# iastro-pt/gpyrn

Measured on AMD Instinct MI355X. Metric: ELBO iterations/sec (N=4096, P=3, Q=2), higher is better.
Workload: dtype f64; 1 GPU; BASELINE config 3: N=4096, p=3 outputs, q=2 nodes, QP nodes / SE weights, synthetic RV series (seed 0); latent_gps=8, comm_ranks=1

## Files before the change

gpyrn_amd/csrc/api.hip:

```cpp
#include "api_internal.h"

#include <dlfcn.h>
#include <fcntl.h>
#include <pthread.h>
#include <sched.h>
#include <sys/mman.h>
#include <sys/stat.h>
#include <time.h>
#include <unistd.h>
#include <atomic>
#include <math.h>
#include <rccl/rccl.h>
#include <stdlib.h>
#include <string.h>

#include <algorithm>

static hipEvent_t prof_event(gprn_ctx* c)
{
    if (!c->prof.pool.empty()) {
        hipEvent_t e = c->prof.pool.back();
        c->prof.pool.pop_back();
        return e;
    }
// ... 123 lines not shown
    if (!c || !name) return GPRN_E_ARG;
    int* field = nullptr;
    if (!strcmp(name, "flags")) { factor_use_flags(c); field = &c->use_flags; }
    else if (!strcmp(name, "wait_budget_ms")) field = &c->wait_budget_ms;
    else if (!strcmp(name, "withhold_inner")) field = &c->withhold_inner;
    else if (!strcmp(name, "overlap")) field = &c->overlap_opt;
    else if (!strcmp(name, "small_path")) field = &c->small_opt;
    else if (!strcmp(name, "bulk_pad_kb")) field = &c->pad_kb_opt;
    else if (!strcmp(name, "small_pad_kb")) field = &c->pad_small_kb_opt;
    else if (!strcmp(name, "batch_mem_mb")) field = &c->batch_mem_mb;
    else if (!strcmp(name, "batch_mask")) field = &c->batch_mask;
    else if (!strcmp(name, "order_mask")) field = &c->order_mask;
    else if (!strcmp(name, "grad_exact")) field = &c->grad_exact;
    else if (!strcmp(name, "elbo_form")) field = &c->elbo_form;
    else if (!strcmp(name, "predict_form")) field = &c->predict_form;
    else if (!strcmp(name, "state_ready")) { if (old) *old = c->grad_ready ? 1 : 0; return GPRN_OK; }
    else if (!strcmp(name, "comm_budget_s")) field = &c->comm_budget_s;
    else if (!strcmp(name, "accurate_factor")) field = &c->acc_opt;
    else if (!strcmp(name, "fenced_finalize")) field = &c->fenced_finalize;
    else if (!strcmp(name, "fallbacks")) { if (old) *old = c->fallbacks; return GPRN_OK; }
    else if (!strcmp(name, "batch_chunk")) { if (old) *old = c->last_batch_chunk; return GPRN_OK; }
    else return bad(c, "set_option: unknown option");
    if (old) *old = *field;
    const bool is_pad = field == &c->pad_kb_opt || field == &c->pad_small_kb_opt;
    if ((is_pad || field == &c->acc_opt) && value == -2) { *field = -1; return GPRN_OK; }
    if (field == &c->predict_form && value < -1)
        return bad(c, "set_option: predict_form is GPRN_PREDICT_REFERENCE or GPRN_PREDICT_POSTERIOR");
    if (value >= 0) {
        if (field == &c->use_flags && value) {
            int can = 0;
            if (hipDeviceGetAttribute(&can, hipDeviceAttributeCanUseStreamWaitValue, c->device) != hipSuccess) can = 0;
            if (!can) return bad(c, "set_option: this device has no stream memory operations");
        }
        if (field == &c->wait_budget_ms && value < 1) return bad(c, "set_option: wait_budget_ms >= 1");
        if (field == &c->batch_mem_mb && value < 1) return bad(c, "set_option: batch_mem_mb >= 1");
        if (field == &c->comm_budget_s && value < 1) return bad(c, "set_option: comm_budget_s >= 1");
        if (field == &c->batch_mask && value > 1) return bad(c, "set_option: batch_mask is 0 or 1");
        if (field == &c->order_mask && value > 1) return bad(c, "set_option: order_mask is 0 or 1");
        if (field == &c->order_mask && !value && c->d_mask && c->sweep_order != GPRN_ORDER_REFERENCE) {
            c->err = "set_option: order_mask stays 1 while a data mask (gprn_set_mask) and the sequential sweep order "
                     "(gprn_set_sweep_order) are both in force";
            return GPRN_E_UNSUPPORTED;
        }
        if (field == &c->grad_exact && value > 1) return bad(c, "set_option: grad_exact is 0 or 1");
        if (field == &c->predict_form) {
            if (value != GPRN_PREDICT_REFERENCE && value != GPRN_PREDICT_POSTERIOR)
                return bad(c, "set_option: predict_form is GPRN_PREDICT_REFERENCE or GPRN_PREDICT_POSTERIOR");
            if (value == GPRN_PREDICT_POSTERIOR && (c->comm || c->shm || c->world > 1)) {
                c->err = "set_option: the posterior form of prediction is not supported on a context with a communicator";
                return GPRN_E_UNSUPPORTED;
            }
        }
        if (field == &c->elbo_form) {
            if (value != GPRN_ELBO_REFERENCE && value != GPRN_ELBO_BOUND) return bad(c, "set_option: elbo_form is GPRN_ELBO_REFERENCE or GPRN_ELBO_BOUND");
            if (value == GPRN_ELBO_BOUND && (c->comm || c->shm || c->world > 1)) {
                c->err = "set_option: the bound form of the ELBO is not supported on a context with a communicator";
                return GPRN_E_UNSUPPORTED;
            }
// ... 39 lines not shown
    HIP_TRY(c, hipMemset(c->d_info, 0, 3 * (size_t)nslot * sizeof(int)));
    c->nslot = nslot;
    return GPRN_OK;
}

void free_problem(gprn_ctx* c)
{
    dev_free(c->d_time); dev_free(c->d_yraw); dev_free(c->d_yerr2); dev_free(c->d_yres);
    dev_free(c->d_variance); dev_free(c->d_mu); dev_free(c->d_var);
    dev_free(c->d_mu_save); dev_free(c->d_var_save);
    dev_free(c->d_mu_alt); dev_free(c->d_var_alt);
    dev_free(c->d_mu_old); c->mu_old_cap = 0;
    if (c->d_loop_ctl) { hipFree(c->d_loop_ctl); c->d_loop_ctl = nullptr; }
    small_batch_free(c);
    mid_batch_free(c);
    if (c->grad_scratch) { hipFree(c->grad_scratch); c->grad_scratch = nullptr; c->grad_scratch_bytes = 0; }
    if (c->h_pin_in) { hipHostFree(c->h_pin_in); c->h_pin_in = nullptr; c->pin_in_cap = 0; }
    if (c->h_pin_out) { hipHostFree(c->h_pin_out); c->h_pin_out = nullptr; c->pin_out_cap = 0; }
    dev_free(c->d_loop_hist);
    for (auto& p : c->K) dev_free(p);
    for (auto& p : c->KLinv) dev_free(p);
    for (auto& p : c->Kinv) dev_free(p);
    for (auto& p : c->Sig) dev_free(p);
    for (auto& p : c->wsB) dev_free(p);
    for (auto& p : c->wsX) dev_free(p);
    c->K.clear(); c->KLinv.clear(); c->Kinv.clear(); c->Sig.clear(); c->wsB.clear(); c->wsX.clear();
    dev_free(c->d_logdetK);
    dev_free(c->d_kinv_tab); dev_free(c->d_kinv_out); dev_free(c->d_small_ticket); dev_free(c->d_small_stamps);
    for (auto& p : c->predKs) dev_free(p);
    for (auto& p : c->predWT) dev_free(p);
// ... 59 lines not shown
{
    if (!out) return GPRN_E_ARG;
    *out = nullptr;
    int n = 0;
    if (hipGetDeviceCount(&n) != hipSuccess || n <= 0) return GPRN_E_NODEV;
    if (device_id < 0 || device_id >= n) return GPRN_E_ARG;
    if (hipSetDevice(device_id) != hipSuccess) return GPRN_E_HIP;
    gprn_ctx* c = new gprn_ctx();
    c->device = device_id;
    c->shared = device_streams_acquire(device_id);
    if (!c->shared) { delete c; return GPRN_E_HIP; }
    c->stream = c->shared->s[0];
    c->stream2 = c->shared->s[1];
    c->stream3 = c->shared->s[2];
    c->stream4 = c->shared->s[3];
    if (hipEventCreateWithFlags(&c->ev_diag, hipEventDisableTiming) != hipSuccess ||
        hipEventCreateWithFlags(&c->ev_first, hipEventDisableTiming) != hipSuccess ||
        hipEventCreateWithFlags(&c->ev_minil, hipEventDisableTiming) != hipSuccess ||
        hipEventCreateWithFlags(&c->ev_inner, hipEventDisableTiming) != hipSuccess ||
        hipEventCreateWithFlags(&c->ev_panel, hipEventDisableTiming) != hipSuccess ||
        hipEventCreateWithFlags(&c->ev_rest, hipEventDisableTiming) != hipSuccess ||
        hipEventCreateWithFlags(&c->ev_resta, hipEventDisableTiming) != hipSuccess ||
        hipEventCreateWithFlags(&c->ev_next, hipEventDisableTiming) != hipSuccess ||
        hipEventCreateWithFlags(&c->ev_nodes, hipEventDisableTiming) != hipSuccess ||
        hipEventCreateWithFlags(&c->ev_tail, hipEventDisableTiming) != hipSuccess ||
        hipEventCreateWithFlags(&c->ev_q1, hipEventDisableTiming) != hipSuccess) {
        device_streams_release(c->shared);
        delete c;
        return GPRN_E_HIP;
    }
// ... 648 lines not shown
```

gpyrn_amd/csrc/api_sweep.hip:

```cpp
#include "api_internal.h"

static int factor_priors_impl(gprn_ctx* c);

extern "C" int gprn_factor_priors(gprn_ctx* c)
{
    DeviceLock lock_(c);
    WatchScope watch_(c, "gprn_factor_priors");
    if (!c || !c->N) return bad(c, "factor_priors: call set_data first");
    HIP_TRY(c, hipSetDevice(c->device));
    if (c->owner.empty()) return bad(c, "factor_priors: call set_owners first");
    c->grad_ready = false;
    int pre = GPRN_OK;
    for (int g = 0; g < c->G && !pre; ++g)
        if (!c->kspec[g].set) pre = bad(c, "factor_priors: a latent GP has no kernel");
    if ((pre = agree_to_start(c, pre, "factor_priors"))) return pre;
    return with_event_fallback(c, "factor_priors", [&](bool) { return factor_priors_impl(c); }, true);
}

static int ensure_small_sweep_tabs(gprn_ctx* c)
{
    if (c->small_sweep_ready) return GPRN_OK;
    std::vector<double*> ktab(c->q, nullptr);
    for (int j = 1; j < c->q && c->elbo_form == GPRN_ELBO_REFERENCE; ++j) {
        if (!c->Kinv[j]) return bad(c, "small path: K_j^-1 of a node is missing (no set-up yet?)");
// ... 200 lines not shown
static int small_sweep(gprn_ctx* c, const double* mu_in, const double* var_in, double* mu_out, double* var_out,
                       double* out4, double* scal, const SmallLoop* loop)
{
    c->d_scal = scal;
    const int* done = loop ? loop->ctl : nullptr;
    TRY(ensure_small_sweep_tabs(c));
    TRY(small_phase(c, sweep_phase(c, false), false, scal, mu_in, var_in, mu_out, var_out, done));
    TRY(order_small(c, sweep_phase(c, false), false, mu_in, var_in, mu_out, var_out, done));
    TRY(mask_rows(c, sweep_phase(c, false), false, mu_out, var_out, done));
    TRY(small_phase(c, sweep_phase(c, true), true, scal, mu_in, var_in, mu_out, var_out, done));
    TRY(order_small(c, sweep_phase(c, true), true, mu_in, var_in, mu_out, var_out, done));
    TRY(mask_rows(c, sweep_phase(c, true), true, mu_out, var_out, done));
    return small_tail(c, out4, scal, mu_out, var_out, loop);
}

int phase_core(gprn_ctx* c, const Phase& ph, bool weights, double* scal, std::function<int()>& chain_started)
{
    const size_t o = (size_t)ph.slot0 * ph.ld;
    TRY(order_snapshot(c, ph));
    TRY(vec_prep(c, ph, weights));
    const int overlap = overlap_mask(c);
    FactorHooks h;
    h.build_B = true;
    h.ft_s = (overlap & 1) ? c->d_s + o : nullptr;
    if (overlap & 2) {
        h.rows_final = [c, &ph, o](int r0, int r1, hipStream_t st) -> int {
            TRY(vec_lower_matvec(c, ph, BUF_X, c->d_z + o, ph.ld, 0, c->d_u + o, st, r0 * GPRN_TILE, (r1 - r0) * GPRN_TILE));
            return vec_colops_partial(c, ph, st, r0, r1 - r0);
        };
    }
    h.chain_started.swap(chain_started);
    const int rc_f = factor_invert(c, ph, false, &h);
    chain_started.swap(h.chain_started);
    TRY(rc_f);
    TRY(vec_lower_matvec(c, ph, BUF_X, c->d_z + o, ph.ld, 0, c->d_u + o, nullptr, h.rows_done * GPRN_TILE, -1));
    TRY(vec_colops_partial(c, ph, nullptr, h.rows_done, -1));
    if (overlap & 8) TRY(vec_reduce_finalize(c, ph, scal, true));
    else {
        TRY(vec_colops_reduce(c, ph));
        TRY(vec_logdet(c, ph, BUF_B, scal));
        TRY(vec_finalize(c, ph, scal, false));
    }
    TRY(order_refresh(c, ph, weights));
    return mask_rows(c, ph, weights, c->d_mu, c->d_var, nullptr);
}

static int mu_k_mu(gprn_ctx* c, bool weights, double* out, hipStream_t stream = nullptr)
{
    const Phase ph = sweep_phase(c, weights);
    if (!ph.nslots) return GPRN_OK;
    double* a = c->d_u + (size_t)ph.slot0 * ph.ld;
    TRY(vec_lower_matvec(c, ph, BUF_KLINV, c->d_mu, c->N, c->elbo_form == GPRN_ELBO_BOUND ? 2 : 1, a, stream));
    return vec_dot_self(c, ph, a, out, stream);
}

struct NodeSide {
    std::function<int()> work;
    bool q1 = false;
    bool term_done = false;
};

static int run_phase(gprn_ctx* c, bool weights, double* scal, std::function<int()>& handed, NodeSide* nodes)
{
    const Phase ph = sweep_phase(c, weights);
    const std::vector<int>& gps = weights ? c->loc_weights : c->loc_nodes;
    const int ns = ph.nslots;
    const size_t o = (size_t)ph.slot0 * ph.ld;
    if (ns) {
        TRY(phase_core(c, ph, weights, scal, handed));
        const int overlap = overlap_mask(c);
        if (c->keep_sigma) {
            const size_t nn = (size_t)c->ld * c->ld;
            TRY(lauum_lower(c, ph));
            for (int s = 0; s < ns; ++s) {
                if (!c->Sig[gps[s]]) {
                    TRY(dev_alloc(c, &c->Sig[gps[s]], nn));
                    HIP_TRY(c, hipMemsetAsync(c->Sig[gps[s]], 0, nn * sizeof(double), c->stream));
                }
                TRY(vec_sigma(c, c->wsB[ph.slot0 + s], c->d_s + o + (size_t)s * c->ld, c->Sig[gps[s]]));
            }
        }
        const bool bound = c->elbo_form == GPRN_ELBO_BOUND;
        if (!weights && c->q > 1 && (!bound || ((overlap & 4) && !c->loc_weights.empty()))) {
            Phase inv = ph;
            inv.nslots = (gps.back() == c->q - 1) ? ns - 1 : ns;
            const std::vector<int> node_gps = gps;
            const std::vector<double*> node_B(c->wsB.begin(), c->wsB.begin() + ns);
            HIP_TRY(c, hipEventRecord(c->ev_nodes, c->stream));
            const bool early_term = (overlap & 4) && !c->loc_weights.empty();
            nodes->term_done = early_term;
            nodes->q1 = true;
            nodes->work = [c, scal, early_term, inv, node_gps, node_B, bound]() -> int {
                HIP_TRY(c, hipStreamWaitEvent(c->stream2, c->ev_nodes, 0));
                if (early_term) TRY(mu_k_mu(c, false, scal + 2 * (size_t)c->G, c->stream2));
                if (inv.nslots && !c->keep_sigma && !bound) TRY(lauum_lower(c, inv, c->stream2));
                for (size_t s = 0; s < node_gps.size() && !bound; ++s) {
                    const int k = node_gps[s];
                    for (int j = k + 1; j < c->q; ++j)
                        TRY(vec_q1(c, c->Kinv[j], node_B[s], c->d_s + s * c->ld, c->d_u,
                                   scal + 3 * (size_t)c->G + (size_t)j * c->q + k, c->stream2));
                }
                HIP_TRY(c, hipEventRecord(c->ev_q1, c->stream2));
                return GPRN_OK;
            };
        }
    }
    if (handed) {
        std::function<int()> f;
        f.swap(handed);
        TRY(f());
    }
    return exchange_rows(c, weights);
}

// ... 458 lines not shown
```

gpyrn_amd/csrc/factor.hip:

```cpp
#include "gprn_internal.h"
#include "tile_mma.h"
#include "diag_tile.h"
#include "vecops.h"

#include <math.h>
#include <stdlib.h>

#include <algorithm>
#include <functional>

template <bool ARGS, bool ACC>
__global__ __launch_bounds__(256) __attribute__((amdgpu_waves_per_eu(1, 1)))
void k_diag_block(double* const* __restrict__ ptrs, PtrArgs pa, int ld, int kblk, int* __restrict__ info,
                  unsigned* sig_slot, unsigned sig_value, const unsigned* wait_flag, unsigned wait_value,
                  unsigned* wait_timed_out, int nph)
{
    __shared__ __attribute__((aligned(16))) double lds[ACC ? DIAG_LDS_DOUBLES_ACC : DIAG_LDS_DOUBLES];
    if (pa.stamps && blockIdx.x == 0 && threadIdx.x == 0) pa.stamps[0] = __builtin_amdgcn_s_memrealtime();
    await_flag(wait_flag, wait_value, wait_timed_out);
    if (pa.stamps && blockIdx.x == 0 && threadIdx.x == 0) pa.stamps[1] = __builtin_amdgcn_s_memrealtime();
    const int slot = blockIdx.x;
    const size_t off = ((size_t)kblk * GPRN_TILE) * ld + (size_t)kblk * GPRN_TILE;
    double* const Bm = ARGS ? pa.p[slot][0] : ptrs[(size_t)slot * GPRN_NBUF + BUF_B];
    double* const Xm = ARGS ? pa.p[slot][1] : ptrs[(size_t)slot * GPRN_NBUF + BUF_X];
// ... 154 lines not shown
                auto by_klen = [](const TileTask& a, const TileTask& b) { return a.klen < b.klen; };
                std::stable_sort(v.begin() + begin, v.begin() + begin + na, by_klen);
                std::stable_sort(v.begin() + begin + na, v.end(), by_klen);
                o.rest0 = begin; o.nrest = v.size() - begin; o.nrestA = na;
            }
        }
        outers.push_back(o);
    }
    }
    c->lauum0 = v.size();
    for (int a = T - 1; a >= 0; --a)
        for (int b = 0; b <= a; ++b)
            v.push_back(TileTask{toff(a, b, ld), toff(a, a, ld), toff(a, b, ld), ld - a * GPRN_TILE,
                                 BUF_B, BUF_X, BUF_X, tile_modes(CM_SET, 1, 1)});
    c->nlauum = v.size() - c->lauum0;

    if (v.size() > c->tasks_cap) {
        if (c->d_tasks) hipFree(c->d_tasks);
        c->d_tasks = nullptr;
        HIP_TRY(c, hipMalloc(&c->d_tasks, v.size() * sizeof(TileTask)));
        c->tasks_cap = v.size();
    }
    HIP_TRY(c, hipStreamSynchronize(c->stream2));
    HIP_TRY(c, hipMemcpyAsync(c->d_tasks, v.data(), v.size() * sizeof(TileTask),
                              hipMemcpyHostToDevice, c->stream));
    HIP_TRY(c, hipStreamSynchronize(c->stream));
    c->tasks_T = T;
    return GPRN_OK;
}

// ... 445 lines not shown
        (void)hipStreamSynchronize(c->stream); (void)hipStreamSynchronize(c->stream2);
        (void)hipStreamSynchronize(c->stream3);
        if (c->stream4) (void)hipStreamSynchronize(c->stream4);
        (void)hipMemset(c->d_sig + (size_t)c->sig_T * GPRN_FLAG_KINDS * 2, 0, sizeof(unsigned));
    }
    return rc;
}

int lauum_lower(gprn_ctx* c, const Phase& ph, hipStream_t stream)
{
    int rc = ensure_tasks(c, ph.T);
    if (rc) return rc;
    return launch_tiles(c, c->d_tasks + c->lauum0, c->nlauum, ph.ptrs, ph.nslots, ph.ld,
                        GPRN_T_LAUUM, stream);
}
```

gpyrn_amd/csrc/gemm_tile.hip:

```cpp
#include "gprn_internal.h"

#include <stdlib.h>
#include <string.h>

#include <algorithm>
#include <type_traits>

#include "tile_mma.h"
#include "diag_tile.h"

template <int BM, int BN, int NW, int TRI, int TAG>
__global__ __launch_bounds__(64 * NW, NW == 8 ? 4 : 2)
void k_tile_gemm(const TileTask* __restrict__ tasks, double* const* __restrict__ ptrs, int ld,
                 unsigned* sig_slot, unsigned sig_value, const unsigned* then_wait, unsigned then_value,
                 const unsigned* wait_flag, unsigned wait_value, unsigned* wait_timed_out, int xcd_map,
                 const double* ft_s, int ft_n,
                 unsigned* start_flag, unsigned start_value, int ldc_arg)
{
    if (start_flag && blockIdx.x == 0 && blockIdx.y == 0 && threadIdx.x == 0)
        __hip_atomic_store(start_flag, start_value, __ATOMIC_RELEASE, __HIP_MEMORY_SCOPE_SYSTEM);
    await_flag(wait_flag, wait_value, wait_timed_out);
    constexpr int WM = 2, WN = NW / 2;
    constexpr int SM = GPRN_TILE / BM, SN = GPRN_TILE / BN;
    __shared__ __attribute__((aligned(16))) double lds[2 * 16 * (BM + BN + 32)];
// ... 5 lines not shown
    const unsigned bx = lb % gx, by = lb / gx;
    const TileTask t = tasks[bx / (SM * SN)];
    const int sub = bx % (SM * SN), sr = sub / SN, sc = sub % SN;
    double* const* gp = ptrs + (size_t)by * GPRN_NBUF;
    double* const p0 = gp[0]; double* const p1 = gp[1]; double* const p2 = gp[2]; double* const p3 = gp[3];
    auto pick = [&](int b) { return b == 0 ? p0 : (b == 1 ? p1 : (b == 2 ? p2 : p3)); };
    const int c_mode = t.modes & 3;
    const int a_mode = (t.modes >> 2) & 1;
    const int b_mode = (t.modes >> 3) & 1;
    const double* A = pick(t.a_buf) + t.a_off + (a_mode ? (size_t)sr * BM : (size_t)sr * BM * ld);
    const double* B = pick(t.b_buf) + t.b_off + (b_mode ? (size_t)sc * BN : (size_t)sc * BN * ld);
    const int ldc_own = TAG == TG_COV ? ldc_arg : 0;
    gptr_t C = (gptr_t)(pick(t.c_buf) + t.c_off) + (size_t)sr * BM * (ldc_own ? ldc_own : ld) + sc * BN;

    constexpr bool CAN_LOWER = BM == 64 && BN == 64 && TRI == 0 &&
                               (TAG == TG_INNER || TAG == TG_NEXT || TAG == TG_BULK || TAG == TG_AHEAD || TAG == TG_COV);
    const bool lower = CAN_LOWER && ((t.modes >> 4) & 1);
    constexpr bool CAN_FT = BM == 64 && BN == 64 && TRI == 0 && (TAG == TG_NEXT || TAG == TG_BULK || TAG == TG_AHEAD);
    const double* ft_K = nullptr;
    const double* ft_sv = nullptr;
    int ft_row = 0, ft_col = 0;
    if (CAN_FT && ft_s && ((t.modes >> 5) & 1)) {
        ft_K = pick(BUF_K) + t.c_off + (size_t)sr * BM * ld + sc * BN;
        ft_sv = ft_s + (size_t)by * ld;
        ft_row = (int)(t.c_off / ld) + sr * BM;
        ft_col = (int)(t.c_off % ld) + sc * BN;
    }
    constexpr bool CAN_SYM128 = BM == 128 && BN == 128 && TRI == 0 && (TAG == TG_INNER || TAG == TG_NEXT);
    if (lower && sr < sc) {  }
    else if (CAN_LOWER && lower && sr == sc)
        tile_mma<BM, BN, WM, WN, TRI, CAN_LOWER, true>(lds, A, B, C, ld, a_mode, b_mode, c_mode, t.klen,
                                                       (sr * BM) >> 4, (sc * BN) >> 4, ft_K, ft_sv, ft_row, ft_col, ft_n, ldc_own);
    else if (CAN_SYM128 && ((t.modes >> 4) & 1))
        tile_mma<BM, BN, WM, WN, TRI, false, false, CAN_SYM128>(lds, A, B, C, ld, a_mode, b_mode, c_mode, t.klen,
                                                                (sr * BM) >> 4, (sc * BN) >> 4);
    else
        tile_mma<BM, BN, WM, WN, TRI, false, true>(lds, A, B, C, ld, a_mode, b_mode, c_mode, t.klen,
                                                   (sr * BM) >> 4, (sc * BN) >> 4, ft_K, ft_sv, ft_row, ft_col, ft_n, ldc_own);
    signal_done(sig_slot, sig_value, then_wait, then_value, wait_timed_out);
}

template <bool ACC>
__global__ __launch_bounds__(256, ACC ? 1 : 2)
void k_tile_panel(const TileTask* __restrict__ tasks, int n_l, double* const* __restrict__ ptrs, int ld,
                  unsigned* sig_slot, unsigned sig_value, const unsigned* then_wait, unsigned then_value,
                  unsigned* wait_timed_out, const unsigned* wait_flag, unsigned wait_value,
                  unsigned* start_flag, unsigned start_value, unsigned* start_flag2)
{
    if (blockIdx.x == 0 && blockIdx.y == 0 && threadIdx.x == 0) {
        if (start_flag) __hip_atomic_store(start_flag, start_value, __ATOMIC_RELEASE, __HIP_MEMORY_SCOPE_SYSTEM);
        if (start_flag2) __hip_atomic_store(start_flag2, start_value, __ATOMIC_RELEASE, __HIP_MEMORY_SCOPE_SYSTEM);
    }
// ... 238 lines not shown
    case TS_64x128_BTRI * 8 + TG_PANEL: GO(64, 128, 1, TG_PANEL); break;
    case TS_128x64_ATRI * 8 + TG_PANEL: GO(128, 64, 2, TG_PANEL); break;
    case TS_64x64 * 8 + TG_INNER: GO(64, 64, 0, TG_INNER); break;
    case TS_128x128 * 8 + TG_INNER: GO(128, 128, 0, TG_INNER); break;
    case TS_64x64 * 8 + TG_NEXT: GO(64, 64, 0, TG_NEXT); break;
    case TS_128x128 * 8 + TG_NEXT: GO(128, 128, 0, TG_NEXT); break;
    case TS_64x64 * 8 + TG_BULK: GO(64, 64, 0, TG_BULK); break;
    case TS_128x128 * 8 + TG_BULK: GO(128, 128, 0, TG_BULK); break;
    case TS_64x64 * 8 + TG_AHEAD: GO(64, 64, 0, TG_AHEAD); break;
    case TS_128x128 * 8 + TG_AHEAD: GO(128, 128, 0, TG_AHEAD); break;
    case TS_128x128 * 8 + TG_MISC: GO(128, 128, 0, TG_MISC); break;
    case TS_64x64 * 8 + TG_MISC: GO(64, 64, 0, TG_MISC); break;
    case TS_64x128 * 8 + TG_MISC: GO(64, 128, 0, TG_MISC); break;
    case TS_128x64 * 8 + TG_MISC: GO(128, 64, 0, TG_MISC); break;
    case TS_64x64 * 8 + TG_COV: GO(64, 64, 0, TG_COV); break;
    default: known = false;
    }
#undef GO
    prof_end(c);
    if (!known) { c->err = "launch_tiles: no kernel for this shape/tag"; return GPRN_E_ARG; }
    if (!fits) return GPRN_E_ARG;
    HIP_TRY(c, hipGetLastError());
    return GPRN_OK;
}

__global__ __launch_bounds__(256, 2)
void k_mfma_peak(double* __restrict__ out, int iters)
{
    v4d acc[16];
#pragma unroll
// ... 38 lines not shown
```

gpyrn_amd/csrc/gprn_internal.h:

```cpp
#pragma once
#include <hip/hip_runtime.h>
#include <stdint.h>
#include <algorithm>
#include <chrono>
#include <functional>
#include <string>
#include <map>
#include <mutex>
#include <vector>

#include "../../include/gprn_hip.h"
#include "batch_layout.h"

#define GPRN_TILE 128
#define GPRN_KC 16
#define GPRN_NBUF 4
#define GPRN_OUTER 4
#define GPRN_OUTER_SMALL 16
#define GPRN_LAT_MAX 32
#define GPRN_FEW_TASKS 4000
#ifndef GPRN_WIDE_CHAIN
#define GPRN_WIDE_CHAIN 48
#endif
#define GPRN_XCD_CHUNK_LOG2 4

#if defined(__gfx942__) || defined(__gfx950__) || !defined(__HIP_DEVICE_COMPILE__)
#define GPRN_RELAXED_HANDOVER 1
#else
#define GPRN_RELAXED_HANDOVER 0
#endif

#define GPRN_GLOBAL __attribute__((address_space(1)))
typedef GPRN_GLOBAL double* gptr_t;
typedef const GPRN_GLOBAL double* gcptr_t;

enum { BUF_B = 0, BUF_X = 1, BUF_K = 2, BUF_KLINV = 3 };
enum { CM_SET = 0, CM_SUB = 1, CM_SETNEG = 2 };

struct TileTask {
    int64_t c_off, a_off, b_off;
    int32_t klen;
    uint8_t c_buf, a_buf, b_buf;
    uint8_t modes;
};
static inline uint8_t tile_modes(int c_mode, int a_mode, int b_mode, int lower_only = 0) {
    return (uint8_t)((c_mode & 3) | ((a_mode & 1) << 2) | ((b_mode & 1) << 3) | ((lower_only & 1) << 4));
}

#define HIP_TRY(ctx, expr)                                                     \
    do {                                                                       \
        hipError_t e_ = (expr);                                                \
        if (e_ != hipSuccess) {                                                \
// ... 125 lines not shown
    std::string last_timeout;
    int pad_kb_opt = -1, pad_small_kb_opt = -1;
    int sig_budget_ms = -1;
    unsigned long long* d_step_stamps = nullptr;
    int step_stamps_T = 0, step_stamps_n = 0;
    int step_stamps_batch[8] = {0};
    unsigned long long *d_side_stamps = nullptr, *side_stamps = nullptr;
    int side_stamps_ph = -1;
    size_t tasks_cap = 0;
    std::vector<TileTask> h_tasks;
    struct StepRange { size_t panel0, npanel_l, npanel, upd0, nupd, ncol1; };
    std::vector<StepRange> steps[2];
    struct OuterRange { int k0, k1; size_t first0, nfirst, next0, nnext, rest0, nrest, nrestA; };
    std::vector<OuterRange> outers[2];
    size_t lauum0 = 0, nlauum = 0;
    int tasks_T = 0;
    int overlap_opt = -1;
    uint8_t* d_mask = nullptr;
    std::vector<uint8_t> h_mask;
    std::vector<std::vector<int>> mask_U;
    int mask_upad = 0;
    int* d_mask_U = nullptr;
    int* d_mask_nU = nullptr;
    std::vector<double*> mask_WT, mask_C;
    double **tab_mask[2] = {nullptr, nullptr};
    int *d_mask_slot[2] = {nullptr, nullptr};
    int *d_mask_gp[2] = {nullptr, nullptr};
    int mask_n[2] = {0, 0};
    TileTask *d_mask_tasks[2] = {nullptr, nullptr};
    size_t mask_ntasks[2] = {0, 0};
// ... 64 lines not shown
bool fill_program_with(const KernelSpec& ks, const double* params, void* dst, double nugget_val);
int launch_fill_batch(gprn_ctx* c, const void* d_programs, double* const* d_Ks, int n_matrices,
                      double* const* d_K2s = nullptr,
                      const double* const* d_diags = nullptr);
int launch_fill_rect_batch(gprn_ctx* c, const void* d_programs, double* const* d_Ks, int n_matrices, const double* d_tstar,
                           int ns, int ns_pad, double* kss, size_t kss_stride);
int launch_fill_rect_batch_post(gprn_ctx* c, const void* d_programs, const char* h_programs, double* const* d_Ks, int n_matrices,
                                const double* d_tstar, int ns, int ns_pad, const double* s, double* kss, size_t kss_stride);
int launch_fill_rect(gprn_ctx* c, const KernelSpec& ks, double nugget_val, const double* d_tstar,
                     int ns, int ns_pad, double* Ks, double* kss);
int launch_fill_rect_post(gprn_ctx* c, const KernelSpec& ks, double nugget_val, const double* d_tstar,
                          int ns, int ns_pad, const double* s, double* Ks, double* kss);
int launch_fill_coincide(gprn_ctx* c, double* K, const double* t, int N, int ld);
enum { TS_128x128 = 0, TS_64x64 = 1, TS_64x128 = 2, TS_128x64 = 3,
       TS_64x128_BTRI = 4, TS_128x64_ATRI = 5 };
enum { TG_PANEL = 0, TG_INNER = 1, TG_NEXT = 2, TG_BULK = 3, TG_MISC = 4, TG_AHEAD = 5, TG_COV = 6 };
struct Signal {
    unsigned* slot; unsigned value;
    const unsigned* then_wait; unsigned then_value; unsigned* timed_out;
};
struct Await { const unsigned* flag; unsigned value; unsigned* timed_out; };
size_t lds_limit(int device);
struct TileSide {
    bool acc = false;
    const double* ft_s = nullptr;
    int N = 0;
    unsigned* start_flag = nullptr;
    unsigned start_value = 0;
    int ldc = 0;
};
int launch_tiles(gprn_ctx* c, const TileTask* d_tasks, size_t ntasks, double** d_ptrs,
// ... 72 lines not shown
            if (value) __hip_atomic_store(slot + 1, value, __ATOMIC_RELEASE, __HIP_MEMORY_SCOPE_SYSTEM);
            if (then_wait) spin_until(then_wait, then_value, timed_out);
        }
    }
}
#endif
struct FactorHooks {
    bool build_B = false;
    const double* ft_s = nullptr;
    std::function<int(int r0, int r1, hipStream_t stream)> rows_final;
    int rows_done = 0;
    std::function<int()> chain_started;
};
int factor_invert(gprn_ctx* c, const Phase& ph, bool prior = false, FactorHooks* hooks = nullptr);
int lauum_lower(gprn_ctx* c, const Phase& ph, hipStream_t stream = nullptr);
int ensure_tasks(gprn_ctx* c, int T);
#define GPRN_E_WAIT_TIMEOUT (-100)
int factor_check_waits(gprn_ctx* c);
int factor_use_flags(gprn_ctx* c);
bool small_applies(const gprn_ctx* c);
int small_phase(gprn_ctx* c, const Phase& ph, bool weights, double* scal, const double* mu_in, const double* var_in,
                double* mu_out, double* var_out, const int* done = nullptr);
struct SmallLoop { int* ctl; double *hist, *last3; int sweep, hist_at, max_iter; };
int small_tail(gprn_ctx* c, double* out4, double* scal, const double* mu, const double* var, const SmallLoop* loop = nullptr);
int small_prior(gprn_ctx* c, double** d_tab, const int* d_job_gp, double** d_kinv_out, int njobs, int* d_info);
struct BatchPred {
    int ns = 0; const double* tstar = nullptr;
    double *lat_mean = nullptr, *lat_var = nullptr, *out_mean = nullptr, *out_var = nullptr;
    int G = 0, p = 0;
    BatchPred from(int e0) const
// ... 86 lines not shown
    int n; const double* kparams; int n_kpar; const double *mu, *var, *jitters; int ns; const double* tstar;
    double *lat_mean, *lat_var, *out_mean, *out_var;
    int* info;
    int p, G; size_t state;
    PredBatchIo slice(int e0, int ne) const
    {
        const size_t lat = (size_t)e0 * G * ns, out = (size_t)e0 * p * ns;
        return PredBatchIo{ne, kparams + (size_t)e0 * n_kpar, n_kpar, mu + e0 * state, var + e0 * state,
                           jitters ? jitters + (size_t)e0 * p : nullptr, ns, tstar,
                           lat_mean ? lat_mean + lat : nullptr, lat_var ? lat_var + lat : nullptr,
                           out_mean ? out_mean + out : nullptr, out_var ? out_var + out : nullptr, info + e0, p, G, state};
    }
};
int mid_predict_run(gprn_ctx* c, const PredBatchIo& io);
int mid_predict_fill_test(gprn_ctx* c, const PredBatchIo& io, int eval, int gp, double* K_out, double* Ks_out, double* kss_out);
int phase_core(gprn_ctx* c, const Phase& ph, bool weights, double* scal, std::function<int()>& chain_started);
int mask_rows(gprn_ctx* c, const Phase& ph, bool weights, double* mu, double* var, const int* done);
int mask_rows_lanes(gprn_ctx* c, const MaskBatch& mb, int N, int ld);
std::vector<int> batch_mask_entries(const gprn_ctx* c, bool weights);
static inline MaskBatch mask_batch_of(const gprn_ctx* c, int ph)
{ return MaskBatch{nullptr, nullptr, 0, c->mask_upad_ph[ph], c->d_mask_tasks[ph], c->mask_ntasks[ph], c->d_mask_U, c->d_mask_nU, c->mask_upad}; }
int mask_prepare(gprn_ctx* c);
void mask_free(gprn_ctx* c);
void mask_invalidate(gprn_ctx* c);

int order_snapshot(gprn_ctx* c, const Phase& ph);
int order_refresh(gprn_ctx* c, const Phase& ph, bool weights);
int order_small(gprn_ctx* c, const Phase& ph, bool weights, const double* mu_in, const double* var_in,
                double* mu_out, double* var_out, const int* done);
int order_small_batch(gprn_ctx* c, const void* lanes, bool weights, int n_eval, bool masked);

// ... 31 lines not shown
```

gpyrn_amd/csrc/tile_mma.h:

```cpp
#pragma once
#include "gprn_internal.h"

#include <type_traits>

typedef double v4d __attribute__((ext_vector_type(4)));
typedef double v2d __attribute__((ext_vector_type(2)));

typedef unsigned v4u __attribute__((ext_vector_type(4)));

#ifndef GPRN_DEEP_PREFETCH
#define GPRN_DEEP_PREFETCH 1
#endif

template <int R, int NT>
__device__ __forceinline__ void lane_geometry(int tid, int mode, int ld, unsigned& goff, int& l0)
{
    constexpr int P = R + 16;
    constexpr int RL = (R < NT / 4) ? R : NT / 4;
    static_assert(R * 8 >= NT && (RL == 64 || RL == 128), "unsupported tile / workgroup combination");
    if (mode == 0) {
        const int kp = tid & 3, row = (tid >> 2) & (RL - 1);
        goff = ((unsigned)row * (unsigned)ld + 2u * kp) * 8u;
        l0 = (2 * kp) * P + (row ^ (4 * kp));
    } else {
        const int rp = tid & (RL / 2 - 1), k = tid / (RL / 2);
        goff = ((unsigned)k * (unsigned)ld + 2u * rp) * 8u;
        l0 = k * P + ((2 * rp) ^ (4 * ((k >> 1) & 3)));
    }
}

template <int BM, int BN, int WM, int WN, int TRI, bool LOWER = false, bool DEEP_OK = false, bool SYM = LOWER>
__device__ __forceinline__ void tile_mma(double* lds, const double* A, const double* B, gptr_t C, int ld,
                                         int a_mode, int b_mode, int c_mode, int klen, int mb16_0, int nb16_0,
                                         const double* ft_K = nullptr,
                                         const double* ft_s = nullptr, int ft_row = 0, int ft_col = 0, int ft_n = 0,
                                         int ldc_own = 0)
{
    const int ldc = ldc_own ? ldc_own : ld;
    const int tid = threadIdx.x;
    const int lane = tid & 63;
    const int wave = __builtin_amdgcn_readfirstlane(tid >> 6);
    const int wr = wave / WN, wc = wave % WN;
    constexpr int NT = 64 * WM * WN;
    constexpr int TM = BM / WM, TN = BN / WN;
    constexpr int MI = TM / 16, NI = TN / 16;
    constexpr int PA = BM + 16, PB = BN + 16;
// ... 15 lines not shown
    const unsigned b_row64 = (b_mode ? 64u : 64u * (unsigned)ld) * 8u, b_k8 = (b_mode ? 8u * (unsigned)ld : 8u) * 8u;
    const int fr = lane & 15, fk = lane >> 4;
    const int mb16 = mb16_0 + ((wr * TM) >> 4), nb16 = nb16_0 + ((wc * TN) >> 4);
    const int row0 = wr * TM;
    int a_fb[4], b_fb[4];
#pragma unroll
    for (int ks = 0; ks < 4; ++ks) {
        const int k = 4 * ks + fk, sw = fr ^ (4 * ((k >> 1) & 3));
        a_fb[ks] = (k * PA + row0 + sw) * 8;
        b_fb[ks] = (A_DOUBLES + k * PB + wc * TN + sw) * 8;
    }
    const char* const lds_b = reinterpret_cast<const char*>(lds);
    char* const lds_w = reinterpret_cast<char*>(lds);
    auto frag = [&](int byte_addr) { return *reinterpret_cast<const double*>(lds_b + byte_addr); };

    const bool neg = c_mode != CM_SET;
    auto on_diag = [&](int i, int j) { return SYM && nb16 + j == mb16 + i; };
    gptr_t Cw = C + (size_t)(row0 + fk) * ldc + wc * TN + fr;
    auto crow = [&](int i) { return (size_t)(i * 16); };
    auto arow_bytes = [&](int i) { return i * 128; };
    v4d acc[MI][NI];

    const int nchunks = klen / GPRN_KC;
    constexpr bool DEEP = DEEP_OK && WM == 2 && WN == 2 &&
                          ((GPRN_DEEP_PREFETCH >= 1 && BM == 64 && BN == 64) || (GPRN_DEEP_PREFETCH >= 2 && BM * BN == 64 * 128));
    v2d ra[A_IT], rb[B_IT];
    v2d ra2[DEEP ? A_IT : 1], rb2[DEEP ? B_IT : 1];
    auto load_chunk = [&](v2d (&ra)[A_IT], v2d (&rb)[B_IT]) {
        const __amdgpu_buffer_rsrc_t ra_rsrc = __builtin_amdgcn_make_buffer_rsrc((void*)A, 0, 0x7fffffff, 0x00020000);
        const __amdgpu_buffer_rsrc_t rb_rsrc = __builtin_amdgcn_make_buffer_rsrc((void*)B, 0, 0x7fffffff, 0x00020000);
#pragma unroll
// ... 42 lines not shown
                    double v = (n < ft_n) ? sm * sc[j] * kv : 0.0;
                    if (m == n) v += 1.0;
                    acc[i][j][r] = on_diag(i, j) ? 0.0 : -v;
                }
            }
    } else if (c_mode == CM_SUB) {
#pragma unroll
        for (int i = 0; i < MI; ++i)
#pragma unroll
            for (int j = 0; j < NI; ++j) {
                if (on_diag(i, j)) { acc[i][j] = v4d{0.0, 0.0, 0.0, 0.0}; continue; }
#pragma unroll
                for (int r = 0; r < 4; ++r)
                    acc[i][j][r] = -Cw[(crow(i) + 4 * r) * ldc + j * 16];
            }
    } else {
#pragma unroll
        for (int i = 0; i < MI; ++i)
#pragma unroll
            for (int j = 0; j < NI; ++j) acc[i][j] = v4d{0.0, 0.0, 0.0, 0.0};
    }
    __builtin_amdgcn_sched_barrier(0);
    write_chunk(0, ra, rb);
    if (nchunks > 1) { A += a_step; B += b_step; }
    load_chunk(ra, rb);
    if constexpr (DEEP) {
        if (nchunks > 2) { A += a_step; B += b_step; }
        load_chunk(ra2, rb2);
    }
    __syncthreads();
// ... 115 lines not shown
```

Measured before the change: 118.9 sweeps/s.

## Compute node inverse product panel-by-panel as factor rows finalize

Splits the LAUUM-style product used by the q1 terms into per-outer-panel tile lists, and launches each one from the rows_final hook as soon as that panel of the inverse is final. This overlaps the product with the rest of the node-phase factorization instead of running it afterwards on stream2. The product goes into new dedicated buffers, and a CM_ADD accumulate mode is added to the tile GEMM. The cost is extra memory, more kernel launches, and possible contention with the critical chain. It is on by default and can be turned off with an option or environment variable.

```diff
diff --git a/gpyrn_amd/csrc/api.hip b/gpyrn_amd/csrc/api.hip
--- a/gpyrn_amd/csrc/api.hip
+++ b/gpyrn_amd/csrc/api.hip
@@ -161,6 +161,7 @@
     else if (!strcmp(name, "grad_exact")) field = &c->grad_exact;
     else if (!strcmp(name, "elbo_form")) field = &c->elbo_form;
     else if (!strcmp(name, "predict_form")) field = &c->predict_form;
+    else if (!strcmp(name, "q1_panels")) field = &c->q1_panels_opt;
     else if (!strcmp(name, "state_ready")) { if (old) *old = c->grad_ready ? 1 : 0; return GPRN_OK; }
     else if (!strcmp(name, "comm_budget_s")) field = &c->comm_budget_s;
     else if (!strcmp(name, "accurate_factor")) field = &c->acc_opt;
@@ -189,6 +190,7 @@
                      "(gprn_set_sweep_order) are both in force";
             return GPRN_E_UNSUPPORTED;
         }
+        if (field == &c->q1_panels_opt && value > 1) return bad(c, "set_option: q1_panels is 0 or 1");
         if (field == &c->grad_exact && value > 1) return bad(c, "set_option: grad_exact is 0 or 1");
         if (field == &c->predict_form) {
             if (value != GPRN_PREDICT_REFERENCE && value != GPRN_PREDICT_POSTERIOR)
@@ -258,6 +260,7 @@
     if (c->d_loop_ctl) { hipFree(c->d_loop_ctl); c->d_loop_ctl = nullptr; }
     small_batch_free(c);
     mid_batch_free(c);
+    q1_free(c);
     if (c->grad_scratch) { hipFree(c->grad_scratch); c->grad_scratch = nullptr; c->grad_scratch_bytes = 0; }
     if (c->h_pin_in) { hipHostFree(c->h_pin_in); c->h_pin_in = nullptr; c->pin_in_cap = 0; }
     if (c->h_pin_out) { hipHostFree(c->h_pin_out); c->h_pin_out = nullptr; c->pin_out_cap = 0; }
@@ -347,6 +350,7 @@
     c->stream2 = c->shared->s[1];
     c->stream3 = c->shared->s[2];
     c->stream4 = c->shared->s[3];
+    if (const char* e = getenv("GPRN_Q1_PANELS")) c->q1_panels_opt = atoi(e) != 0 ? 1 : 0;
     if (hipEventCreateWithFlags(&c->ev_diag, hipEventDisableTiming) != hipSuccess ||
         hipEventCreateWithFlags(&c->ev_first, hipEventDisableTiming) != hipSuccess ||
         hipEventCreateWithFlags(&c->ev_minil, hipEventDisableTiming) != hipSuccess ||
diff --git a/gpyrn_amd/csrc/api_sweep.hip b/gpyrn_amd/csrc/api_sweep.hip
--- a/gpyrn_amd/csrc/api_sweep.hip
+++ b/gpyrn_amd/csrc/api_sweep.hip
@@ -238,7 +238,7 @@
     return small_tail(c, out4, scal, mu_out, var_out, loop);
 }
 
-int phase_core(gprn_ctx* c, const Phase& ph, bool weights, double* scal, std::function<int()>& chain_started)
+int phase_core(gprn_ctx* c, const Phase& ph, bool weights, double* scal, std::function<int()>& chain_started, Q1Panels* q1)
 {
     const size_t o = (size_t)ph.slot0 * ph.ld;
     TRY(order_snapshot(c, ph));
@@ -248,9 +248,18 @@
     h.build_B = true;
     h.ft_s = (overlap & 1) ? c->d_s + o : nullptr;
     if (overlap & 2) {
-        h.rows_final = [c, &ph, o](int r0, int r1, hipStream_t st) -> int {
+        h.rows_final = [c, &ph, o, q1](int r0, int r1, hipStream_t st) -> int {
             TRY(vec_lower_matvec(c, ph, BUF_X, c->d_z + o, ph.ld, 0, c->d_u + o, st, r0 * GPRN_TILE, (r1 - r0) * GPRN_TILE));
-            return vec_colops_partial(c, ph, st, r0, r1 - r0);
+            TRY(vec_colops_partial(c, ph, st, r0, r1 - r0));
+            if (!q1) return GPRN_OK;
+            const std::vector<gprn_ctx::OuterRange>& outers = c->outers[q1->set];
+            if ((size_t)q1->done >= outers.size() || outers[(size_t)q1->done].k0 != r0 || outers[(size_t)q1->done].k1 != r1) {
+                c->err = "phase_core: rows_final left the order of the outer panels";
+                return GPRN_E_ARG;
+            }
+            TRY(lauum_panels(c, q1->ph, q1->set, q1->done, q1->done + 1, st));
+            q1->done += 1;
+            return GPRN_OK;
         };
     }
     h.chain_started.swap(chain_started);
@@ -278,6 +287,54 @@
     return vec_dot_self(c, ph, a, out, stream);
 }
 
+struct Q1Buffers {
+    DeviceOwner mem;
+    std::vector<double*> buf, X;
+    double** tab = nullptr;
+    int ld = 0;
+    bool failed = false;
+};
+
+void q1_free(gprn_ctx* c)
+{
+    delete (Q1Buffers*)c->q1_mem;
+    c->q1_mem = nullptr;
+}
+
+static Q1Buffers* q1_ensure(gprn_ctx* c, int n)
+{
+    Q1Buffers* q = (Q1Buffers*)c->q1_mem;
+    const std::vector<double*> X(c->wsX.begin(), c->wsX.begin() + n);
+    if (q && q->ld == c->ld && q->X == X) return q->failed ? nullptr : q;
+    q1_free(c);
+    q = new Q1Buffers();
+    c->q1_mem = q;
+    q->ld = c->ld;
+    q->X = X;
+    const size_t nn = (size_t)c->ld * c->ld;
+    std::vector<double*> rows((size_t)n * GPRN_NBUF, nullptr);
+    bool ok = true;
+    for (int s = 0; s < n && ok; ++s) {
+        double* b = nullptr;
+        ok = q->mem.alloc(c, &b, nn) == GPRN_OK && hipMemsetAsync(b, 0, nn * sizeof(double), c->stream2) == hipSuccess;
+        q->buf.push_back(b);
+        rows[(size_t)s * GPRN_NBUF + BUF_B] = b;
+        rows[(size_t)s * GPRN_NBUF + BUF_X] = X[(size_t)s];
+    }
+    ok = ok && q->mem.alloc(c, &q->tab, rows.size()) == GPRN_OK &&
+         hipMemcpy(q->tab, rows.data(), rows.size() * sizeof(double*), hipMemcpyHostToDevice) == hipSuccess;
+    if (!ok) {
+        (void)hipGetLastError();
+        (void)hipStreamSynchronize(c->stream2);
+        q->mem.release();
+        q->buf.clear();
+        q->tab = nullptr;
+        q->failed = true;
+        return nullptr;
+    }
+    return q;
+}
+
 struct NodeSide {
     std::function<int()> work;
     bool q1 = false;
@@ -291,8 +348,15 @@
     const int ns = ph.nslots;
     const size_t o = (size_t)ph.slot0 * ph.ld;
     if (ns) {
-        TRY(phase_core(c, ph, weights, scal, handed));
         const int overlap = overlap_mask(c);
+        const int n_inv = weights ? 0 : ((gps.back() == c->q - 1) ? ns - 1 : ns);
+        Q1Panels q1{ph, ph.nslots * ph.T <= GPRN_LAT_MAX ? 1 : 0, 0};
+        Q1Buffers* q1b = nullptr;
+        if (!weights && c->q > 1 && n_inv > 0 && c->q1_panels_opt != 0 && (overlap & 2) && !c->keep_sigma &&
+            c->elbo_form != GPRN_ELBO_BOUND)
+            q1b = q1_ensure(c, n_inv);
+        if (q1b) { q1.ph.ptrs = q1b->tab; q1.ph.nslots = n_inv; }
+        TRY(phase_core(c, ph, weights, scal, handed, q1b ? &q1 : nullptr));
         if (c->keep_sigma) {
             const size_t nn = (size_t)c->ld * c->ld;
             TRY(lauum_lower(c, ph));
@@ -314,14 +378,18 @@
             const bool early_term = (overlap & 4) && !c->loc_weights.empty();
             nodes->term_done = early_term;
             nodes->q1 = true;
-            nodes->work = [c, scal, early_term, inv, node_gps, node_B, bound]() -> int {
+            const Q1Panels q1_rest = q1;
+            const std::vector<double*> q1_B = q1b ? q1b->buf : std::vector<double*>();
+            const int q1_end = q1b ? (int)c->outers[q1.set].size() : 0;
+            nodes->work = [c, scal, early_term, inv, node_gps, node_B, bound, q1_rest, q1_B, q1_end]() -> int {
                 HIP_TRY(c, hipStreamWaitEvent(c->stream2, c->ev_nodes, 0));
                 if (early_term) TRY(mu_k_mu(c, false, scal + 2 * (size_t)c->G, c->stream2));
-                if (inv.nslots && !c->keep_sigma && !bound) TRY(lauum_lower(c, inv, c->stream2));
+                if (!q1_B.empty()) TRY(lauum_panels(c, q1_rest.ph, q1_rest.set, q1_rest.done, q1_end, c->stream2));
+                else if (inv.nslots && !c->keep_sigma && !bound) TRY(lauum_lower(c, inv, c->stream2));
                 for (size_t s = 0; s < node_gps.size() && !bound; ++s) {
                     const int k = node_gps[s];
                     for (int j = k + 1; j < c->q; ++j)
-                        TRY(vec_q1(c, c->Kinv[j], node_B[s], c->d_s + s * c->ld, c->d_u,
+                        TRY(vec_q1(c, c->Kinv[j], s < q1_B.size() ? q1_B[s] : node_B[s], c->d_s + s * c->ld, c->d_u,
                                    scal + 3 * (size_t)c->G + (size_t)j * c->q + k, c->stream2));
                 }
                 HIP_TRY(c, hipEventRecord(c->ev_q1, c->stream2));
diff --git a/gpyrn_amd/csrc/factor.hip b/gpyrn_amd/csrc/factor.hip
--- a/gpyrn_amd/csrc/factor.hip
+++ b/gpyrn_amd/csrc/factor.hip
@@ -192,6 +192,19 @@
             v.push_back(TileTask{toff(a, b, ld), toff(a, a, ld), toff(a, b, ld), ld - a * GPRN_TILE,
                                  BUF_B, BUF_X, BUF_X, tile_modes(CM_SET, 1, 1)});
     c->nlauum = v.size() - c->lauum0;
+    for (int set = 0; set < 2; ++set) {
+        c->q1_lists[set].clear();
+        for (const gprn_ctx::OuterRange& o : c->outers[set]) {
+            const size_t begin = v.size();
+            for (int a = o.k1 - 1; a >= 0; --a)
+                for (int b = 0; b <= a; ++b) {
+                    const int r0 = std::max(a, o.k0);
+                    v.push_back(TileTask{toff(a, b, ld), toff(r0, a, ld), toff(r0, b, ld), (o.k1 - r0) * GPRN_TILE,
+                                         BUF_B, BUF_X, BUF_X, tile_modes(a >= o.k0 ? CM_SET : CM_ADD, 1, 1, a == b)});
+                }
+            c->q1_lists[set].push_back(gprn_ctx::ListRange{begin, v.size() - begin});
+        }
+    }
 
     if (v.size() > c->tasks_cap) {
         if (c->d_tasks) hipFree(c->d_tasks);
@@ -667,3 +680,16 @@
     return launch_tiles(c, c->d_tasks + c->lauum0, c->nlauum, ph.ptrs, ph.nslots, ph.ld,
                         GPRN_T_LAUUM, stream);
 }
+
+int lauum_panels(gprn_ctx* c, const Phase& ph, int set, int J0, int J1, hipStream_t stream)
+{
+    int rc = ensure_tasks(c, ph.T);
+    if (rc) return rc;
+    const std::vector<gprn_ctx::ListRange>& lists = c->q1_lists[set];
+    if (J0 < 0 || J1 > (int)lists.size()) { c->err = "lauum_panels: no such outer panel"; return GPRN_E_ARG; }
+    for (int J = J0; J < J1; ++J)
+        if ((rc = launch_tiles(c, c->d_tasks + lists[(size_t)J].first, lists[(size_t)J].n, ph.ptrs, ph.nslots, ph.ld, GPRN_T_LAUUM,
+                               stream, TS_64x64, Signal{nullptr, 0, nullptr, 0, nullptr}, Await{nullptr, 0, nullptr}, TG_Q1)))
+            return rc;
+    return GPRN_OK;
+}
diff --git a/gpyrn_amd/csrc/gemm_tile.hip b/gpyrn_amd/csrc/gemm_tile.hip
--- a/gpyrn_amd/csrc/gemm_tile.hip
+++ b/gpyrn_amd/csrc/gemm_tile.hip
@@ -43,7 +43,8 @@
     gptr_t C = (gptr_t)(pick(t.c_buf) + t.c_off) + (size_t)sr * BM * (ldc_own ? ldc_own : ld) + sc * BN;
 
     constexpr bool CAN_LOWER = BM == 64 && BN == 64 && TRI == 0 &&
-                               (TAG == TG_INNER || TAG == TG_NEXT || TAG == TG_BULK || TAG == TG_AHEAD || TAG == TG_COV);
+                               (TAG == TG_INNER || TAG == TG_NEXT || TAG == TG_BULK || TAG == TG_AHEAD || TAG == TG_COV || TAG == TG_Q1);
+    constexpr bool ADD_OK = TAG == TG_Q1;
     const bool lower = CAN_LOWER && ((t.modes >> 4) & 1);
     constexpr bool CAN_FT = BM == 64 && BN == 64 && TRI == 0 && (TAG == TG_NEXT || TAG == TG_BULK || TAG == TG_AHEAD);
     const double* ft_K = nullptr;
@@ -58,13 +59,13 @@
     constexpr bool CAN_SYM128 = BM == 128 && BN == 128 && TRI == 0 && (TAG == TG_INNER || TAG == TG_NEXT);
     if (lower && sr < sc) {  }
     else if (CAN_LOWER && lower && sr == sc)
-        tile_mma<BM, BN, WM, WN, TRI, CAN_LOWER, true>(lds, A, B, C, ld, a_mode, b_mode, c_mode, t.klen,
+        tile_mma<BM, BN, WM, WN, TRI, CAN_LOWER, true, CAN_LOWER && !ADD_OK, ADD_OK>(lds, A, B, C, ld, a_mode, b_mode, c_mode, t.klen,
                                                        (sr * BM) >> 4, (sc * BN) >> 4, ft_K, ft_sv, ft_row, ft_col, ft_n, ldc_own);
     else if (CAN_SYM128 && ((t.modes >> 4) & 1))
         tile_mma<BM, BN, WM, WN, TRI, false, false, CAN_SYM128>(lds, A, B, C, ld, a_mode, b_mode, c_mode, t.klen,
                                                                 (sr * BM) >> 4, (sc * BN) >> 4);
     else
-        tile_mma<BM, BN, WM, WN, TRI, false, true>(lds, A, B, C, ld, a_mode, b_mode, c_mode, t.klen,
+        tile_mma<BM, BN, WM, WN, TRI, false, true, false, ADD_OK>(lds, A, B, C, ld, a_mode, b_mode, c_mode, t.klen,
                                                    (sr * BM) >> 4, (sc * BN) >> 4, ft_K, ft_sv, ft_row, ft_col, ft_n, ldc_own);
     signal_done(sig_slot, sig_value, then_wait, then_value, wait_timed_out);
 }
@@ -333,6 +334,7 @@
     case TS_64x128 * 8 + TG_MISC: GO(64, 128, 0, TG_MISC); break;
     case TS_128x64 * 8 + TG_MISC: GO(128, 64, 0, TG_MISC); break;
     case TS_64x64 * 8 + TG_COV: GO(64, 64, 0, TG_COV); break;
+    case TS_64x64 * 8 + TG_Q1: GO(64, 64, 0, TG_Q1); break;
     default: known = false;
     }
 #undef GO
diff --git a/gpyrn_amd/csrc/gprn_internal.h b/gpyrn_amd/csrc/gprn_internal.h
--- a/gpyrn_amd/csrc/gprn_internal.h
+++ b/gpyrn_amd/csrc/gprn_internal.h
@@ -35,7 +35,8 @@
 typedef const GPRN_GLOBAL double* gcptr_t;
 
 enum { BUF_B = 0, BUF_X = 1, BUF_K = 2, BUF_KLINV = 3 };
-enum { CM_SET = 0, CM_SUB = 1, CM_SETNEG = 2 };
+enum { CM_SET = 0, CM_SUB = 1, CM_SETNEG = 2,
+       CM_ADD = 3 };
 
 struct TileTask {
     int64_t c_off, a_off, b_off;
@@ -191,6 +192,10 @@
     struct OuterRange { int k0, k1; size_t first0, nfirst, next0, nnext, rest0, nrest, nrestA; };
     std::vector<OuterRange> outers[2];
     size_t lauum0 = 0, nlauum = 0;
+    struct ListRange { size_t first, n; };
+    std::vector<ListRange> q1_lists[2];
+    int q1_panels_opt = 1;
+    void* q1_mem = nullptr;
     int tasks_T = 0;
     int overlap_opt = -1;
     uint8_t* d_mask = nullptr;
@@ -285,7 +290,7 @@
 int launch_fill_coincide(gprn_ctx* c, double* K, const double* t, int N, int ld);
 enum { TS_128x128 = 0, TS_64x64 = 1, TS_64x128 = 2, TS_128x64 = 3,
        TS_64x128_BTRI = 4, TS_128x64_ATRI = 5 };
-enum { TG_PANEL = 0, TG_INNER = 1, TG_NEXT = 2, TG_BULK = 3, TG_MISC = 4, TG_AHEAD = 5, TG_COV = 6 };
+enum { TG_PANEL = 0, TG_INNER = 1, TG_NEXT = 2, TG_BULK = 3, TG_MISC = 4, TG_AHEAD = 5, TG_COV = 6, TG_Q1 = 7 };
 struct Signal {
     unsigned* slot; unsigned value;
     const unsigned* then_wait; unsigned then_value; unsigned* timed_out;
@@ -388,6 +393,8 @@
 };
 int factor_invert(gprn_ctx* c, const Phase& ph, bool prior = false, FactorHooks* hooks = nullptr);
 int lauum_lower(gprn_ctx* c, const Phase& ph, hipStream_t stream = nullptr);
+int lauum_panels(gprn_ctx* c, const Phase& ph, int set, int J0, int J1, hipStream_t stream);
+void q1_free(gprn_ctx* c);
 int ensure_tasks(gprn_ctx* c, int T);
 #define GPRN_E_WAIT_TIMEOUT (-100)
 int factor_check_waits(gprn_ctx* c);
@@ -504,7 +511,9 @@
 };
 int mid_predict_run(gprn_ctx* c, const PredBatchIo& io);
 int mid_predict_fill_test(gprn_ctx* c, const PredBatchIo& io, int eval, int gp, double* K_out, double* Ks_out, double* kss_out);
-int phase_core(gprn_ctx* c, const Phase& ph, bool weights, double* scal, std::function<int()>& chain_started);
+struct Q1Panels { Phase ph; int set; int done; };
+int phase_core(gprn_ctx* c, const Phase& ph, bool weights, double* scal, std::function<int()>& chain_started,
+               Q1Panels* q1 = nullptr);
 int mask_rows(gprn_ctx* c, const Phase& ph, bool weights, double* mu, double* var, const int* done);
 int mask_rows_lanes(gprn_ctx* c, const MaskBatch& mb, int N, int ld);
 std::vector<int> batch_mask_entries(const gprn_ctx* c, bool weights);
diff --git a/gpyrn_amd/csrc/tile_mma.h b/gpyrn_amd/csrc/tile_mma.h
--- a/gpyrn_amd/csrc/tile_mma.h
+++ b/gpyrn_amd/csrc/tile_mma.h
@@ -29,7 +29,7 @@
     }
 }
 
-template <int BM, int BN, int WM, int WN, int TRI, bool LOWER = false, bool DEEP_OK = false, bool SYM = LOWER>
+template <int BM, int BN, int WM, int WN, int TRI, bool LOWER = false, bool DEEP_OK = false, bool SYM = LOWER, bool ADD_OK = false>
 __device__ __forceinline__ void tile_mma(double* lds, const double* A, const double* B, gptr_t C, int ld,
                                          int a_mode, int b_mode, int c_mode, int klen, int mb16_0, int nb16_0,
                                          const double* ft_K = nullptr,
@@ -75,7 +75,7 @@
     char* const lds_w = reinterpret_cast<char*>(lds);
     auto frag = [&](int byte_addr) { return *reinterpret_cast<const double*>(lds_b + byte_addr); };
 
-    const bool neg = c_mode != CM_SET;
+    const bool neg = ADD_OK ? (c_mode == CM_SUB || c_mode == CM_SETNEG) : c_mode != CM_SET;
     auto on_diag = [&](int i, int j) { return SYM && nb16 + j == mb16 + i; };
     gptr_t Cw = C + (size_t)(row0 + fk) * ldc + wc * TN + fr;
     auto crow = [&](int i) { return (size_t)(i * 16); };
@@ -148,6 +148,14 @@
                 for (int r = 0; r < 4; ++r)
                     acc[i][j][r] = -Cw[(crow(i) + 4 * r) * ldc + j * 16];
             }
+    } else if (ADD_OK && c_mode == CM_ADD) {
+#pragma unroll
+        for (int i = 0; i < MI; ++i)
+#pragma unroll
+            for (int j = 0; j < NI; ++j)
+#pragma unroll
+                for (int r = 0; r < 4; ++r)
+                    acc[i][j][r] = Cw[(crow(i) + 4 * r) * ldc + j * 16];
     } else {
 #pragma unroll
         for (int i = 0; i < MI; ++i)
diff --git a/profiles/q1_panels_timing.py b/profiles/q1_panels_timing.py
--- /dev/null
+++ b/profiles/q1_panels_timing.py
@@ -0,0 +1,71 @@
+import argparse
+import json
+import os
+import subprocess
+import sys
+
+import numpy as np
+
+HERE = os.path.dirname(os.path.dirname(os.path.abspath(__file__)))
+
+
+def bench(env_extra, args):
+    env = dict(os.environ)
+    env.pop('GPRN_HIP_LIB', None)
+    env.pop('GPRN_Q1_PANELS', None)
+    env.update(env_extra)
+    r = subprocess.run([sys.executable, 'bench.py'] + args, cwd=HERE, env=env, capture_output=True, text=True, timeout=400)
+    if r.returncode:
+        raise RuntimeError('bench.py %s under %s ended with status %d: %s' % (' '.join(args), env_extra, r.returncode, r.stderr[-400:]))
+    row = [json.loads(ln) for ln in r.stdout.splitlines() if ln.startswith('{')][-1]
+    if row['schedule']['fallbacks'] or row['info']:
+        raise RuntimeError('bench.py under %s: fallbacks %s, info %s' % (env_extra, row['schedule']['fallbacks'], row['info']))
+    return {'ms_per_sweep': row['ms_per_step'], 'sweeps_per_s': row['value'], 'blocks': row['blocks']['sweeps_per_s'],
+            'elbo_last': row['elbo_last'], 'flags': row['schedule']['flags']}
+
+
+def main():
+    ap = argparse.ArgumentParser()
+    ap.add_argument('--parent-lib', required=True)
+    ap.add_argument('--out', default='q1_panels_timing.json')
+    ap.add_argument('--rounds', type=int, default=9)
+    ap.add_argument('--config4', action='store_true')
+    a = ap.parse_args()
+    legs = [('parent', {'GPRN_HIP_LIB': os.path.abspath(a.parent_lib)}), ('off', {'GPRN_Q1_PANELS': '0'}), ('on', {'GPRN_Q1_PANELS': '1'})]
+    head = ['--gpus', '1', '--steps', '20', '--warmup', '3', '--blocks', '20']
+    res = {'command': 'bench.py ' + ' '.join(head), 'rounds': a.rounds, 'runs': {n: [] for n, _ in legs}}
+    failed = None
+    try:
+        for r in range(a.rounds):
+            for name, env in legs:
+                res['runs'][name].append(bench(env, head))
+            print('round', r + 1, {n: round(res['runs'][n][-1]['ms_per_sweep'], 4) for n, _ in legs}, flush=True)
+        ms = {n: [x['ms_per_sweep'] for x in rs] for n, rs in res['runs'].items()}
+        res['ms_per_sweep'] = {n: {'median': float(np.median(v)), 'min': min(v), 'max': max(v)} for n, v in ms.items()}
+        pm = res['ms_per_sweep']['parent']
+        spread = (pm['max'] - pm['min']) / pm['median']
+        res['parent_rel_spread_min_max'] = spread
+        res['off_over_parent'] = res['ms_per_sweep']['off']['median'] / pm['median']
+        res['on_over_parent'] = res['ms_per_sweep']['on']['median'] / pm['median']
+        res['on_over_off'] = res['ms_per_sweep']['on']['median'] / res['ms_per_sweep']['off']['median']
+        res['same_elbo_every_run'] = len({x['elbo_last'] for rs in res['runs'].values() for x in rs}) == 1
+        res['condition_1_off_equals_parent_within_its_spread'] = bool(abs(res['off_over_parent'] - 1.0) <= spread)
+        res['condition_2_on_faster_than_parent_by_more_than_its_spread'] = bool(1.0 - res['on_over_parent'] > spread)
+        if a.config4:
+            c4 = ['--config', '4', '--gpus', '1', '--steps', '10', '--warmup', '2', '--blocks', '5']
+            res['config4'] = {'command': 'bench.py ' + ' '.join(c4), 'off': [], 'on': []}
+            for _ in range(2):
+                for name, env in legs[1:]:
+                    res['config4'][name].append(bench(env, c4))
+            print('config 4', {n: [round(x['ms_per_sweep'], 3) for x in res['config4'][n]] for n in ('off', 'on')}, flush=True)
+    except BaseException as e:
+        failed = '%s: %s' % (type(e).__name__, e)
+        res['error'] = failed
+    with open(a.out, 'w') as f:
+        json.dump(res, f, indent=1)
+    print(json.dumps({k: v for k, v in res.items() if k != 'runs'}), flush=True)
+    sys.exit(1 if failed else 0)
+
+
+if __name__ == '__main__':
+    main()
diff --git a/profiles/q1_panels_trace.py b/profiles/q1_panels_trace.py
--- /dev/null
+++ b/profiles/q1_panels_trace.py
@@ -0,0 +1,48 @@
+#!/usr/bin/env python3
+import csv
+import glob
+import re
+import statistics as st
+import sys
+
+d = sys.argv[1]
+f = glob.glob(d + '/**/*kernel_trace.csv', recursive=True)[0]
+rows = []
+for r in csv.DictReader(open(f)):
+    rows.append((int(r['Start_Timestamp']), int(r['End_Timestamp']), re.sub(r'\s+', '', r['Kernel_Name'].split('(')[0].replace('void ', ''))))
+rows.sort()
+Q1 = ('k_tile_gemm<64,64,4,0,7>', 'k_tile_gemm<128,128,8,0,4>')
+CHAIN = ('k_diag_block', 'k_chain_l', 'k_chain_u')
+pn = [i for i, r in enumerate(rows) if r[2].startswith('k_prep_nodes')]
+pw = [i for i, r in enumerate(rows) if r[2].startswith('k_prep_weights')]
+out = []
+for n, a in enumerate(pn[:-1]):
+    w = [i for i in pw if i > a]
+    nxt = pn[n + 1]
+    if not w or w[0] > nxt or rows[nxt][0] - rows[a][0] > 50e6:
+        continue
+    t0, tw, t1 = rows[a][0], rows[w[0]][0], rows[nxt][0]
+    node = [k for k in rows[a:w[0]]]
+    diag = sorted(k[0] for k in node if k[2].startswith('k_diag_block'))
+    chain_end = max(k[1] for k in node if k[2].startswith(CHAIN))
+    prod = [k for k in rows[a:nxt] if k[2].startswith(Q1)]
+    if not diag or not prod:
+        continue
+    steps = [(y - x) / 1e3 for x, y in zip(diag[:-1], diag[1:])]
+    out.append({'n': len(prod), 'sum': sum(k[1] - k[0] for k in prod) / 1e3,
+                'in_node': sum(max(0, min(k[1], tw) - k[0]) for k in prod if k[0] < tw) / 1e3,
+                'launches': [((k[0] - diag[0]) / 1e3, (k[1] - diag[0]) / 1e3) for k in prod],
+                'chain_end': (chain_end - diag[0]) / 1e3, 'node_end': (tw - diag[0]) / 1e3,
+                'step_median': st.median(steps), 'step_sum': sum(steps), 'sweep': (t1 - t0) / 1e3})
+print('%d kernels, %d sweeps with a product' % (len(rows), len(out)))
+if out:
+    med = lambda key: st.median(x[key] for x in out)
+    print('product launches per sweep %d | summed duration %.1f us | of it inside the node phase %.1f us' % (med('n'), med('sum'), med('in_node')))
+    print('node phase, from its first diagonal block: last chain kernel ends %.1f us | k_prep_weights starts %.1f us' % (med('chain_end'), med('node_end')))
+    print('node phase chain step (diag to diag): median %.1f us | sum over the phase %.1f us | sweep %.1f us' % (med('step_median'), med('step_sum'), med('sweep')))
+    nl = int(med('n'))
+    same = [x for x in out if x['n'] == nl]
+    for j in range(nl):
+        print('  product launch %d: start %8.1f  end %8.1f  (%.1f us)' % (j, st.median(x['launches'][j][0] for x in same),
+                                                                          st.median(x['launches'][j][1] for x in same),
+                                                                          st.median(x['launches'][j][1] - x['launches'][j][0] for x in same)))
```

Result: no change. 118.6 sweeps/s, median of 4 (-0.2%).
